# Chengyuann/AutoStyle-TTS

Hardware: AMD Instinct MI355X
Metric: synthesized audio sec/wall-sec (RTF^-1) + style-kNN QPS, IEMOCAP test batch (higher is better)
Workload: dtype f16; 1 GPU; BASELINE configs[1]: batch=8 utterances/GPU, kNN Q=8 x N=1000 x D=6144 k=3, synthesis Tt=32 Tp=150 Ts=250 (fixed-length decode, EOS ignored) -> 430 mel frames -> 110080 samples @ 22050 Hz; CosyVoice-300M shapes, random-init weights; parallelism=dp1 (model + bank replicated, utterances sharded, all-gather of style ids only)

## Files before the change

### autostyle-tts_amd/csrc/ops_tfm_fused.hip

```cpp
#include "common.h"
#include "xlane.h"

namespace astts {

static constexpr int TF_C = 256;
static constexpr int TF_DH = 64;
static constexpr int TF_KS = 72;
static constexpr int TF_AS = TF_C + 8;
static constexpr int TF_QROWS = 192;
static constexpr int TF_QS = 64;
static constexpr int TF_MAX_T = 384;

__device__ __forceinline__ int tf_q(int row, int col) { return row * TF_QS + ((((col >> 3) ^ row) & 7) << 3) + (col & 7); }

__device__ __forceinline__ float row16_sum(float v) {
    v += __builtin_bit_cast(float, __builtin_amdgcn_update_dpp(0, __builtin_bit_cast(int, v), 0x121, 0xf, 0xf, false));
    v += __builtin_bit_cast(float, __builtin_amdgcn_update_dpp(0, __builtin_bit_cast(int, v), 0x122, 0xf, 0xf, false));
    v += __builtin_bit_cast(float, __builtin_amdgcn_update_dpp(0, __builtin_bit_cast(int, v), 0x124, 0xf, 0xf, false));
    v += __builtin_bit_cast(float, __builtin_amdgcn_update_dpp(0, __builtin_bit_cast(int, v), 0x128, 0xf, 0xf, false));
    return v;
}

struct TfmAttnArgs {
    const float* x;
    const _Float16* w;
    const float* bias;
    const int* lens;
    _Float16* out;
    int b, heads, t;
    float eps, scale;
    int balance;
    const char* pf[3];
    unsigned pf_bytes[4];
};

template <bool FULL>
__device__ __forceinline__ void tfm_attn_body(const TfmAttnArgs& a, int* seq_out, int* unit_out) {
    extern __shared__ __attribute__((aligned(16))) _Float16 tf_smem[];
    const int tid = threadIdx.x, lane = tid & 63, wid = tid >> 6;
    const int c = lane & 31, hh = lane >> 5;
    int qs, head, b;
    {
        const int units = FULL ? a.heads : 2 * a.heads;
        const int L = blockIdx.x;
        int hq;
        if ((a.b & 7) == 0) {
            const int xcd = L & 7, slot = L >> 3;
            b = xcd + 8 * (slot / units);
            hq = slot % units;
        } else {
            b = L / units;
            hq = L % units;
        }
        head = FULL ? hq : hq >> 1;
        qs = FULL ? 0 : hq & 1;
    }
    const int T = a.t;
    const int nch = (T + 31) >> 5;
    const int tkp = nch * 32;
    const int vs = tkp + 4;
    const int hsplit = (nch + 1) / 2;
    const int pq0 = FULL ? 0 : (qs == 0 ? 0 : hsplit);
    const int pq1 = FULL ? nch : (qs == 0 ? hsplit : nch);
    _Float16* sK = tf_smem;
    _Float16* sVt = sK + (size_t)tkp * TF_KS;
    _Float16* sA = sVt + (size_t)TF_DH * vs;
    _Float16* sQ = sA + 2 * 32 * TF_AS;
    const float* xb = a.x + (int64_t)b * T * TF_C;
    const int hd = a.heads * TF_DH;

    const int role = wid >> 1;
    half8 wf[16];
    float bias_e[16];
    if (role < 3) {
        const int part = role == 0 ? 1 : (role == 1 ? 2 : 0);
        const int frow = part * hd + head * TF_DH + (wid & 1) * 32;
        const _Float16* wp = a.w + ((int64_t)(frow >> 5) * 16 * 64 + lane) * 8;
#pragma unroll
        for (int s = 0; s < 16; ++s) wf[s] = *reinterpret_cast<const half8*>(wp + (int64_t)s * 64 * 8);
#pragma unroll
        for (int e = 0; e < 16; ++e) {
            const int f = role == 1 ? c : (e & 3) + 8 * (e >> 2) + 4 * hh;
            bias_e[e] = a.bias ? a.bias[frow + f] : 0.0f;
        }
    }

    const int srow = tid >> 4, sseg = (tid & 15) * 16;
    constexpr int PF = 2;
    float4 xr[PF][4];
    auto load_chunk = [&](int ch, float4 (&r)[4]) {
        const int fr = min(ch * 32 + srow, T - 1);
        const float* p = xb + (int64_t)fr * TF_C + sseg;
#pragma unroll
        for (int i = 0; i < 4; ++i) r[i] = *reinterpret_cast<const float4*>(p + 4 * i);
    };
    auto stage_chunk = [&](int buf, const float4 (&r)[4]) {
        float s = 0.0f;
#pragma unroll
        for (int i = 0; i < 4; ++i) s += (r[i].x + r[i].y) + (r[i].z + r[i].w);
        s = row16_sum(s);
        const float mean = s * (1.0f / TF_C);
        float q = 0.0f;
#pragma unroll
        for (int i = 0; i < 4; ++i) {
            const float dx = r[i].x - mean, dy = r[i].y - mean, dz = r[i].z - mean, dw = r[i].w - mean;
            q += (dx * dx + dy * dy) + (dz * dz + dw * dw);
        }
        q = row16_sum(q);
        const float rstd = rsqrtf(q * (1.0f / TF_C) + a.eps);
        half8 h0, h1;
        h0[0] = (_Float16)((r[0].x - mean) * rstd); h0[1] = (_Float16)((r[0].y - mean) * rstd);
        h0[2] = (_Float16)((r[0].z - mean) * rstd); h0[3] = (_Float16)((r[0].w - mean) * rstd);
        h0[4] = (_Float16)((r[1].x - mean) * rstd); h0[5] = (_Float16)((r[1].y - mean) * rstd);
        h0[6] = (_Float16)((r[1].z - mean) * rstd); h0[7] = (_Float16)((r[1].w - mean) * rstd);
        h1[0] = (_Float16)((r[2].x - mean) * rstd); h1[1] = (_Float16)((r[2].y - mean) * rstd);
        h1[2] = (_Float16)((r[2].z - mean) * rstd); h1[3] = (_Float16)((r[2].w - mean) * rstd);
        h1[4] = (_Float16)((r[3].x - mean) * rstd); h1[5] = (_Float16)((r[3].y - mean) * rstd);
        h1[6] = (_Float16)((r[3].z - mean) * rstd); h1[7] = (_Float16)((r[3].w - mean) * rstd);
        _Float16* d = sA + (size_t)buf * 32 * TF_AS + srow * TF_AS + sseg;
        *reinterpret_cast<half8*>(d) = h0;
        *reinterpret_cast<half8*>(d + 8) = h1;
    };
    auto project_chunk = [&](int ch) {
        const int buf = ch & 1;
        const bool q_chunk = ch >= pq0 && ch < pq1;
        const bool q_parked = FULL && ch >= hsplit;
        const int qbase = FULL ? 0 : pq0;
        if (role < 2 || (role == 2 && q_chunk)) {
            const _Float16* ap = sA + (size_t)buf * 32 * TF_AS + c * TF_AS + 8 * hh;
            float16v acc;
#pragma unroll
            for (int e = 0; e < 16; ++e) acc[e] = bias_e[e];
            if (role == 1) {
#pragma unroll
                for (int s0 = 0; s0 < 16; s0 += 8) {
                    half8 af[8];
#pragma unroll
                    for (int s = 0; s < 8; ++s) af[s] = *reinterpret_cast<const half8*>(ap + 16 * (s0 + s));
#pragma unroll
                    for (int s = 0; s < 8; ++s) acc = __builtin_amdgcn_mfma_f32_32x32x16_f16(af[s], wf[s0 + s], acc, 0, 0, 0);
                }
                _Float16* vp = sVt + (size_t)((wid & 1) * 32 + c) * vs + ch * 32 + 4 * hh;
#pragma unroll
                for (int g = 0; g < 4; ++g) {
                    half4 h4;
                    h4[0] = (_Float16)acc[4 * g]; h4[1] = (_Float16)acc[4 * g + 1]; h4[2] = (_Float16)acc[4 * g + 2]; h4[3] = (_Float16)acc[4 * g + 3];
                    *reinterpret_cast<half4*>(vp + 8 * g) = h4;
                }
            } else {
#pragma unroll
                for (int s0 = 0; s0 < 16; s0 += 8) {
                    half8 af[8];
#pragma unroll
                    for (int s = 0; s < 8; ++s) af[s] = *reinterpret_cast<const half8*>(ap + 16 * (s0 + s));
#pragma unroll
                    for (int s = 0; s < 8; ++s) acc = __builtin_amdgcn_mfma_f32_32x32x16_f16(wf[s0 + s], af[s], acc, 0, 0, 0);
                }
                _Float16* kp = sK + (size_t)(ch * 32 + c) * TF_KS + (wid & 1) * 32 + 4 * hh;
                const int qr = (ch - qbase) * 32 + c;
                const int fr = ch * 32 + c;
                _Float16* park = a.out + ((int64_t)b * T + min(fr, T - 1)) * hd + head * TF_DH + (wid & 1) * 32 + 4 * hh;
#pragma unroll
                for (int g = 0; g < 4; ++g) {
                    half4 h4;
                    h4[0] = (_Float16)acc[4 * g]; h4[1] = (_Float16)acc[4 * g + 1]; h4[2] = (_Float16)acc[4 * g + 2]; h4[3] = (_Float16)acc[4 * g + 3];
                    if (role == 0) *reinterpret_cast<half4*>(kp + 8 * g) = h4;
                    else if (!q_parked) *reinterpret_cast<half4*>(sQ + tf_q(qr, (wid & 1) * 32 + 4 * hh + 8 * g)) = h4;
                    else if (fr < T) *reinterpret_cast<half4*>(park + 8 * g) = h4;
                }
            }
        }
    };
#pragma unroll
    for (int i = 0; i < PF; ++i)
        if (i < nch) load_chunk(i, xr[i]);
    stage_chunk(0, xr[0]);
    if (PF < nch) load_chunk(PF, xr[0]);
    __syncthreads();
    for (int ch0 = 0; ch0 < nch; ch0 += PF) {
#pragma unroll
        for (int u = 0; u < PF; ++u) {
            const int ch = ch0 + u;
            if (ch < nch) {
                if (ch + 1 < nch) stage_chunk((ch + 1) & 1, xr[(u + 1) % PF]);
                if (ch + 1 + PF < nch) load_chunk(ch + 1 + PF, xr[(u + 1) % PF]);
                project_chunk(ch);
                __syncthreads();
            }
        }
    }

    unsigned pf_keep[3];
    *seq_out = b;
    *unit_out = FULL ? head * 2 : head * 2 + qs;
    for (int hf = FULL ? 0 : qs; hf < (FULL ? 2 : qs + 1); ++hf) {
    const int qch0 = hf == 0 ? 0 : hsplit;
    const int qch1 = hf == 0 ? hsplit : nch;
    if (FULL && hf == 1) {
        __builtin_amdgcn_fence(__ATOMIC_RELEASE, "workgroup");
        __syncthreads();
        __builtin_amdgcn_fence(__ATOMIC_ACQUIRE, "workgroup");
        const int rows = (nch - hsplit) * 32;
        for (int i = tid; i < rows * 8; i += 512) {
            const int r = i >> 3, pc = i & 7;
            const int fr = min(hsplit * 32 + r, T - 1);
            const half8 v = *reinterpret_cast<const half8*>(a.out + ((int64_t)b * T + fr) * hd + head * TF_DH + pc * 8);
            *reinterpret_cast<half8*>(sQ + tf_q(r, pc * 8)) = v;
        }
        __syncthreads();
    }
    const int ntile = qch1 - qch0;
    int tile = -1, part = 0, parts = 1;
    if (wid < 4) {
        if (wid < ntile) tile = wid;
    } else if (!a.balance) {
        if (wid < ntile) tile = wid;
    } else if (ntile == 5) {
        tile = 4; part = wid - 4; parts = 4;
    } else if (ntile == 6) {
        tile = 4 + (wid & 1); part = (wid - 4) >> 1; parts = 2;
    }
    if (hf == (FULL ? 0 : qs)) {
        const unsigned slot = blockIdx.x >> 3, nslots = max(gridDim.x >> 3, 1u);
        asm volatile("" ::"s"(a.pf_bytes[3]));
#pragma unroll
        for (int r = 0; r < 3; ++r) {
            const unsigned lines = a.pf[r] ? (a.pf_bytes[r] + 127) >> 7 : 0u;
            const unsigned per = (lines + nslots - 1) / nslots;
            const unsigned ln = slot * per + tid;
            const char* base = a.pf[r] ? a.pf[r] : reinterpret_cast<const char*>(a.x);
            prefetch_line(base + (tid < per && ln < lines ? (size_t)ln << 7 : (size_t)0), pf_keep[r]);
        }
    }
    const int len = a.lens ? min(a.lens[b], T) : T;
    const int nkt = (len + 31) >> 5;
    const int jb0 = tile >= 0 ? (nkt * part / parts) * 32 : 0;
    const int jb1 = tile >= 0 ? min((nkt * (part + 1) / parts) * 32, len) : 0;
    const int tsafe = tile >= 0 ? tile : 0;
    const int q0 = (qch0 + tsafe) * 32;
    _Float16* qrow = sQ + (size_t)(tsafe * 32) * TF_QS;
    half8 qf[4];
    {
        const float qscale = a.scale * 1.44269504088896341f;
#pragma unroll
        for (int s = 0; s < 4; ++s) {
            const half8 raw = *reinterpret_cast<const half8*>(qrow + tf_q(c, 16 * s + 8 * hh));
#pragma unroll
            for (int i = 0; i < 8; ++i) qf[s][i] = (_Float16)((float)raw[i] * qscale);
        }
    }
    float16v ot[2];
#pragma unroll
    for (int e = 0; e < 16; ++e) {
        ot[0][e] = 0.0f;
        ot[1][e] = 0.0f;
    }
    float m_run = -INFINITY, l_run = 0.0f;
    for (int jb = jb0; jb < jb1; jb += 32) {
        float16v st;
#pragma unroll
        for (int e = 0; e < 16; ++e) st[e] = 0.0f;
        half8 kf[4];
        half4 vlo[4], vhi[4];
#pragma unroll
        for (int s = 0; s < 4; ++s) kf[s] = *reinterpret_cast<const half8*>(sK + (size_t)(jb + c) * TF_KS + 16 * s + 8 * hh);
#pragma unroll
        for (int dt = 0; dt < 2; ++dt)
#pragma unroll
            for (int s = 0; s < 2; ++s) {
                const _Float16* vrow = sVt + (size_t)(dt * 32 + c) * vs + jb + 16 * s + 4 * hh;
                vlo[dt * 2 + s] = *reinterpret_cast<const half4*>(vrow);
                vhi[dt * 2 + s] = *reinterpret_cast<const half4*>(vrow + 8);
            }
#pragma unroll
        for (int s = 0; s < 4; ++s) st = __builtin_amdgcn_mfma_f32_32x32x16_f16(kf[s], qf[s], st, 0, 0, 0);
        if (jb + 32 > len) {
#pragma unroll
            for (int e = 0; e < 16; ++e) {
                const int key = jb + (e & 3) + 8 * (e >> 2) + 4 * hh;
                st[e] = key < len ? st[e] : -INFINITY;
            }
        }
        float mloc = st[0];
#pragma unroll
        for (int e = 1; e < 16; ++e) mloc = fmaxf(mloc, st[e]);
        mloc = fmaxf(mloc, __shfl_xor(mloc, 32, 64));
        if (__builtin_amdgcn_ballot_w64(mloc > m_run) != 0) {
            const float m_new = fmaxf(m_run, mloc);
            const float alpha = __builtin_amdgcn_exp2f(m_run - m_new);
            l_run *= alpha;
            m_run = m_new;
#pragma unroll
            for (int e = 0; e < 16; ++e) {
                ot[0][e] *= alpha;
                ot[1][e] *= alpha;
            }
        }
        half8 pf[2];
#pragma unroll
        for (int e = 0; e < 16; ++e) {
            const float p = __builtin_amdgcn_exp2f(st[e] - m_run);
            l_run += p;
            pf[e >> 3][e & 7] = (_Float16)p;
        }
#pragma unroll
        for (int dt = 0; dt < 2; ++dt) {
#pragma unroll
            for (int s = 0; s < 2; ++s) {
                const half4 lo = vlo[dt * 2 + s], hi = vhi[dt * 2 + s];
                half8 vf;
                vf[0] = lo[0]; vf[1] = lo[1]; vf[2] = lo[2]; vf[3] = lo[3];
                vf[4] = hi[0]; vf[5] = hi[1]; vf[6] = hi[2]; vf[7] = hi[3];
                ot[dt] = __builtin_amdgcn_mfma_f32_32x32x16_f16(vf, pf[s], ot[dt], 0, 0, 0);
            }
        }
    }
    float* sM = reinterpret_cast<float*>(sA);
    if (part > 0) {
        float* mp = sM + (size_t)(ntile == 5 ? part - 1 : wid - 6) * 34 * 64 + lane;
#pragma unroll
        for (int e = 0; e < 16; ++e) {
            mp[e * 64] = ot[0][e];
            mp[(16 + e) * 64] = ot[1][e];
        }
        mp[32 * 64] = m_run;
        mp[33 * 64] = l_run;
    }
    __syncthreads();
    if (!(tile < 0 || part > 0)) {
    for (int hp = 1; hp < parts; ++hp) {
        const float* mp = sM + (size_t)(ntile == 5 ? hp - 1 : wid - 4) * 34 * 64 + lane;
        const float m_p = mp[32 * 64], l_p = mp[33 * 64];
        const float m_new = fmaxf(m_run, m_p);
        if (m_new > -INFINITY) {
            const float sa = __builtin_amdgcn_exp2f(m_run - m_new), sb = __builtin_amdgcn_exp2f(m_p - m_new);
#pragma unroll
            for (int e = 0; e < 16; ++e) {
                ot[0][e] = ot[0][e] * sa + mp[e * 64] * sb;
                ot[1][e] = ot[1][e] * sa + mp[(16 + e) * 64] * sb;
            }
            l_run = l_run * sa + l_p * sb;
            m_run = m_new;
        }
    }
    l_run += __shfl_xor(l_run, 32, 64);
    const float inv = l_run > 0.0f ? 1.0f / l_run : 0.0f;
#pragma unroll
    for (int dt = 0; dt < 2; ++dt)
#pragma unroll
        for (int g = 0; g < 4; ++g) {
            half4 h4;
            h4[0] = (_Float16)(ot[dt][4 * g] * inv); h4[1] = (_Float16)(ot[dt][4 * g + 1] * inv);
            h4[2] = (_Float16)(ot[dt][4 * g + 2] * inv); h4[3] = (_Float16)(ot[dt][4 * g + 3] * inv);
            *reinterpret_cast<half4*>(qrow + tf_q(c, dt * 32 + 8 * g + 4 * hh)) = h4;
        }
    __builtin_amdgcn_s_waitcnt(0xc07f);
    __builtin_amdgcn_wave_barrier();
#pragma unroll
    for (int i = 0; i < 4; ++i) {
        const int r = i * 8 + (lane >> 3), seg = (lane & 7) * 8;
        const int fr = q0 + r;
        if (fr < T)
            *reinterpret_cast<half8*>(a.out + ((int64_t)b * T + fr) * hd + head * TF_DH + seg) = *reinterpret_cast<const half8*>(qrow + tf_q(r, seg));
    }
    }
    }
    prefetch_keep(pf_keep[0]);
    prefetch_keep(pf_keep[1]);
    prefetch_keep(pf_keep[2]);
}

template <bool FULL>
__global__ __launch_bounds__(512, 2) void tfm_attn_fused(const float* p_x, const _Float16* p_w, const float* p_bias, const int* p_lens, int p_b, int p_heads,
                                                         int p_t, float p_eps, float p_scale, TfmAttnArgs a_in) {
    TfmAttnArgs a = a_in;
    a.x = p_x; a.w = p_w; a.bias = p_bias; a.lens = p_lens; a.b = p_b; a.heads = p_heads; a.t = p_t; a.eps = p_eps; a.scale = p_scale;
    int seq, unit;
    tfm_attn_body<FULL>(a, &seq, &unit);
}

__global__ void tfm_pack_frag(const _Float16* __restrict__ w, _Float16* __restrict__ out, int rows, int k) {
    const int64_t total = (int64_t)rows * k;
    const int ksteps = k >> 4;
    for (int64_t i = (int64_t)blockIdx.x * blockDim.x + threadIdx.x; i < total; i += (int64_t)gridDim.x * blockDim.x) {
        const int j = (int)(i & 7), ln = (int)((i >> 3) & 63);
        const int64_t q = i >> 9;
        const int s = (int)(q % ksteps);
        const int64_t tile = q / ksteps;
        out[i] = w[(tile * 32 + (ln & 31)) * k + 16 * s + 8 * (ln >> 5) + j];
    }
}

static constexpr int FF_HS = 256 + 8;

struct TfmFfnArgs {
    const float* x;
    const _Float16* w1;
    const float* b1;
    const _Float16* w2;
    const float* b2;
    float* out;
    const _Float16* attn;
    const _Float16* wo;
    const float* bo;
    int64_t m;
    int hidden, k0;
    float eps;
    const char* pf;
    unsigned pf_bytes;
};

template <bool WO>
__device__ __forceinline__ void tfm_ffn_body(const TfmFfnArgs& a, const int64_t m0, const int64_t mend, const unsigned rot_seed) {
    extern __shared__ __attribute__((aligned(16))) _Float16 tf_smem[];
    const int tid = threadIdx.x, lane = tid & 63, wid = tid >> 6;
    const int c = lane & 31, hh = lane >> 5;
    _Float16* sA = tf_smem;
    _Float16* sH = sA + 32 * TF_AS;
    float* sB1 = reinterpret_cast<float*>(sH + 2 * 32 * FF_HS);
    const int nchunk = a.hidden >> 8;
    const int ksteps2 = a.hidden >> 4;

    const int srow = tid >> 4, sseg = (tid & 15) * 4;
    float4 r[4];
    {
        const float* p = a.x + min(m0 + srow, mend - 1) * TF_C + sseg;
#pragma unroll
        for (int i = 0; i < 4; ++i) r[i] = *reinterpret_cast<const float4*>(p + 64 * i);
    }
    const int rot = (int)(rot_seed % (unsigned)nchunk);
    auto wrap = [&](int j) { return j >= nchunk ? j - nchunk : j; };
    half8 w1f[16], w2f[16];
    const _Float16* w1p = a.w1 + ((int64_t)wid * 16 * 64 + lane) * 8;
    const _Float16* w2p = a.w2 + ((int64_t)wid * ksteps2 * 64 + lane) * 8;
    auto load_w1 = [&](int j) {
        const _Float16* np = w1p + (int64_t)j * 8 * 16 * 512;
#pragma unroll
        for (int s = 0; s < 16; ++s) w1f[s] = *reinterpret_cast<const half8*>(np + (int64_t)s * 512);
    };
    auto load_w2 = [&](int j) {
        const _Float16* np = w2p + (int64_t)j * 16 * 512;
#pragma unroll
        for (int s = 0; s < 16; ++s) w2f[s] = *reinterpret_cast<const half8*>(np + (int64_t)s * 512);
    };
    float* sX = sB1 + a.hidden;
    if constexpr (WO) {
        const int as0 = a.k0 + 8;
        _Float16* sAtt = sH;
        const int nh = a.k0 >> 8;
        const _Float16* wop = a.wo + ((int64_t)wid * (a.k0 >> 4) * 64 + lane) * 8;
        half8 at[4];
        {
            const _Float16* p = a.attn + min(m0 + srow, mend - 1) * a.k0 + (tid & 15) * 8;
#pragma unroll
            for (int i = 0; i < 4; ++i)
                if (i * 128 < a.k0) at[i] = *reinterpret_cast<const half8*>(p + 128 * i);
        }
#pragma unroll
        for (int s = 0; s < 16; ++s) w2f[s] = *reinterpret_cast<const half8*>(wop + (int64_t)s * 512);
        load_w1(rot);
        for (int i = tid; i < a.hidden; i += 512) sB1[i] = a.b1 ? a.b1[i] : 0.0f;
        float16v acc0;
        {
            const float* bp = a.bo + wid * 32 + 4 * hh;
#pragma unroll
            for (int g = 0; g < 4; ++g) {
                const float4 b4 = a.bo ? *reinterpret_cast<const float4*>(bp + 8 * g) : make_float4(0.0f, 0.0f, 0.0f, 0.0f);
                acc0[4 * g] = b4.x; acc0[4 * g + 1] = b4.y; acc0[4 * g + 2] = b4.z; acc0[4 * g + 3] = b4.w;
            }
        }
#pragma unroll
        for (int i = 0; i < 4; ++i) *reinterpret_cast<float4*>(sX + srow * 260 + sseg + 64 * i) = r[i];
#pragma unroll
        for (int i = 0; i < 4; ++i)
            if (i * 128 < a.k0) *reinterpret_cast<half8*>(sAtt + srow * as0 + (tid & 15) * 8 + 128 * i) = at[i];
        __syncthreads();
        const _Float16* atp = sAtt + c * as0 + 8 * hh;
        for (int h = 0; h < nh; ++h) {
#pragma unroll
            for (int s0 = 0; s0 < 16; s0 += 8) {
                half8 af[8];
#pragma unroll
                for (int s = 0; s < 8; ++s) af[s] = *reinterpret_cast<const half8*>(atp + 16 * (16 * h + s0 + s));
#pragma unroll
                for (int s = 0; s < 8; ++s) acc0 = __builtin_amdgcn_mfma_f32_32x32x16_f16(w2f[s0 + s], af[s], acc0, 0, 0, 0);
            }
            if (h + 1 < nh) {
                const _Float16* np = wop + (int64_t)(h + 1) * 16 * 512;
#pragma unroll
                for (int s = 0; s < 16; ++s) w2f[s] = *reinterpret_cast<const half8*>(np + (int64_t)s * 512);
            }
        }
        load_w2(rot);
        {
            float* xp = sX + c * 260 + wid * 32 + 4 * hh;
#pragma unroll
            for (int g = 0; g < 4; ++g) {
                float4 v = *reinterpret_cast<float4*>(xp + 8 * g);
                v.x += acc0[4 * g]; v.y += acc0[4 * g + 1]; v.z += acc0[4 * g + 2]; v.w += acc0[4 * g + 3];
                *reinterpret_cast<float4*>(xp + 8 * g) = v;
            }
        }
        __syncthreads();
#pragma unroll
        for (int i = 0; i < 4; ++i) r[i] = *reinterpret_cast<const float4*>(sX + srow * 260 + sseg + 64 * i);
    } else {
        load_w1(rot);
        load_w2(rot);
        for (int i = tid; i < a.hidden; i += 512) sB1[i] = a.b1 ? a.b1[i] : 0.0f;
    }
    {
        float s = 0.0f;
#pragma unroll
        for (int i = 0; i < 4; ++i) s += (r[i].x + r[i].y) + (r[i].z + r[i].w);
        s = row16_sum(s);
        const float mean = s * (1.0f / TF_C);
        float q = 0.0f;
#pragma unroll
        for (int i = 0; i < 4; ++i) {
            const float dx = r[i].x - mean, dy = r[i].y - mean, dz = r[i].z - mean, dw = r[i].w - mean;
            q += (dx * dx + dy * dy) + (dz * dz + dw * dw);
        }
        q = row16_sum(q);
        const float rstd = rsqrtf(q * (1.0f / TF_C) + a.eps);
        _Float16* d = sA + srow * TF_AS + sseg;
#pragma unroll
        for (int i = 0; i < 4; ++i) {
            half4 h4;
            h4[0] = (_Float16)((r[i].x - mean) * rstd); h4[1] = (_Float16)((r[i].y - mean) * rstd);
            h4[2] = (_Float16)((r[i].z - mean) * rstd); h4[3] = (_Float16)((r[i].w - mean) * rstd);
            *reinterpret_cast<half4*>(d + 64 * i) = h4;
        }
    }
    __syncthreads();

    unsigned pf_keep;
    {
        const unsigned slot = blockIdx.x >> 3, nslots = max((gridDim.x + 7) >> 3, 1u);
        const unsigned lines = a.pf ? (a.pf_bytes + 127) >> 7 : 0u;
        const unsigned per = (lines + nslots - 1) / nslots;
        const unsigned ln = slot * per + tid;
        const char* base = a.pf ? a.pf : reinterpret_cast<const char*>(a.x);
        prefetch_line(base + (tid < per && ln < lines ? (size_t)ln << 7 : (size_t)0), pf_keep);
    }
    float16v acc2;
#pragma unroll
    for (int e = 0; e < 16; ++e) acc2[e] = 0.0f;
    const _Float16* ap = sA + c * TF_AS + 8 * hh;
    auto stage1 = [&](int j, float16v& acc1) {
        const float* bp = sB1 + (j * 8 + wid) * 32 + 4 * hh;
#pragma unroll
        for (int g = 0; g < 4; ++g) {
            const float4 b4 = *reinterpret_cast<const float4*>(bp + 8 * g);
            acc1[4 * g] = b4.x; acc1[4 * g + 1] = b4.y; acc1[4 * g + 2] = b4.z; acc1[4 * g + 3] = b4.w;
        }
#pragma unroll
        for (int s0 = 0; s0 < 16; s0 += 8) {
            half8 af[8];
#pragma unroll
            for (int s = 0; s < 8; ++s) af[s] = *reinterpret_cast<const half8*>(ap + 16 * (s0 + s));
#pragma unroll
            for (int s = 0; s < 8; ++s) acc1 = __builtin_amdgcn_mfma_f32_32x32x16_f16(w1f[s0 + s], af[s], acc1, 0, 0, 0);
        }
    };
    auto store_h = [&](int buf, const float (&gl)[16]) {
        _Float16* hp = sH + (size_t)buf * 32 * FF_HS + c * FF_HS + wid * 32 + 4 * hh;
#pragma unroll
        for (int g = 0; g < 4; ++g) {
            half4 h4;
            h4[0] = (_Float16)gl[4 * g]; h4[1] = (_Float16)gl[4 * g + 1]; h4[2] = (_Float16)gl[4 * g + 2]; h4[3] = (_Float16)gl[4 * g + 3];
            *reinterpret_cast<half4*>(hp + 8 * g) = h4;
        }
    };
    {
        float16v acc1;
        stage1(rot, acc1);
        if (nchunk > 1) load_w1(wrap(rot + 1));
        float gl[16];
#pragma unroll
        for (int e = 0; e < 16; ++e) gl[e] = gelu_erf_fast(acc1[e]);
        store_h(0, gl);
    }
    __syncthreads();
    for (int it = 0; it + 1 < nchunk; ++it) {
        const int jn = wrap(it + 1 + rot);
        float16v acc1;
        stage1(jn, acc1);
        if (it + 2 < nchunk) load_w1(wrap(jn + 1));
        const _Float16* hp = sH + (size_t)(it & 1) * 32 * FF_HS + c * FF_HS + 8 * hh;
        float gl[16];
#pragma unroll
        for (int s0 = 0; s0 < 16; s0 += 8) {
            half8 hf[8];
#pragma unroll
            for (int s = 0; s < 8; ++s) hf[s] = *reinterpret_cast<const half8*>(hp + 16 * (s0 + s));
            __builtin_amdgcn_sched_barrier(0);
#pragma unroll
            for (int s = 0; s < 8; ++s) {
                float gx = acc1[s0 + s];
                asm volatile("" : "+v"(hf[s]), "+v"(gx));
                acc2 = __builtin_amdgcn_mfma_f32_32x32x16_f16(hf[s], w2f[s0 + s], acc2, 0, 0, 0);
                float gy = gelu_erf_fast(gx);
                asm volatile("" : "+v"(gy), "+v"(hf[s]));
                gl[s0 + s] = gy;
                __builtin_amdgcn_sched_barrier(0);
            }
        }
        load_w2(jn);
        store_h((it + 1) & 1, gl);
        __syncthreads();
    }
    const int f = wid * 32 + c;
    float xr[16];
#pragma unroll
    for (int e = 0; e < 16; ++e) {
        const int re = (e & 3) + 8 * (e >> 2) + 4 * hh;
        xr[e] = WO ? sX[re * 260 + f] : a.x[min(m0 + re, mend - 1) * TF_C + f];
    }
    const float b2 = a.b2 ? a.b2[f] : 0.0f;
    {
        const _Float16* hp = sH + (size_t)((nchunk - 1) & 1) * 32 * FF_HS + c * FF_HS + 8 * hh;
#pragma unroll
        for (int s0 = 0; s0 < 16; s0 += 8) {
            half8 hf[8];
#pragma unroll
            for (int s = 0; s < 8; ++s) hf[s] = *reinterpret_cast<const half8*>(hp + 16 * (s0 + s));
#pragma unroll
            for (int s = 0; s < 8; ++s) acc2 = __builtin_amdgcn_mfma_f32_32x32x16_f16(hf[s], w2f[s0 + s], acc2, 0, 0, 0);
        }
    }
#pragma unroll
    for (int e = 0; e < 16; ++e) {
        const int64_t row = m0 + (e & 3) + 8 * (e >> 2) + 4 * hh;
        if (row < mend) a.out[row * TF_C + f] = (xr[e] + b2) + acc2[e];
    }
    prefetch_keep(pf_keep);
}

template <bool WO>
__global__ __launch_bounds__(512, 1) void tfm_ffn_fused(const float* p_x, const _Float16* p_w1, const _Float16* p_attn, const _Float16* p_wo, int64_t p_m,
                                                        int p_hidden, int p_k0, float p_eps, TfmFfnArgs a_in) {
    TfmFfnArgs a = a_in;
    a.x = p_x; a.w1 = p_w1; a.attn = p_attn; a.wo = p_wo; a.m = p_m; a.hidden = p_hidden; a.k0 = p_k0; a.eps = p_eps;
    const int64_t m0 = (int64_t)blockIdx.x * 32;
    tfm_ffn_body<WO>(a, m0, min(m0 + 32, a.m), blockIdx.x >> 3);
}

}

using namespace astts;

extern "C" {

int astts_op_tfm_pack_frag(const void* w_f16, void* out_f16, int32_t rows, int32_t k, astts_stream_t stream) {
    ASTTS_REQUIRE(w_f16 && out_f16 && w_f16 != out_f16, ASTTS_ERR_INVALID, "astts_op_tfm_pack_frag: null / aliased pointer");
    ASTTS_REQUIRE(k >= 16 && k % 16 == 0 && rows >= 32 && rows % 32 == 0, ASTTS_ERR_UNSUPPORTED,
                  "astts_op_tfm_pack_frag: rows=%d k=%d (rows must be a multiple of 32, k of 16)", rows, k);
    hipLaunchKernelGGL(tfm_pack_frag, dim3(256), dim3(256), 0, (hipStream_t)stream, (const _Float16*)w_f16, (_Float16*)out_f16, rows, k);
    ASTTS_CHECK_LAUNCH();
    return ASTTS_OK;
}

int astts_op_tfm_ffn_fused_supported(int32_t c, int32_t hidden) {
    return c == TF_C && hidden >= 256 && hidden % 256 == 0 && hidden <= 4096 ? 1 : 0;
}

int astts_op_tfm_ffn_fused(const float* x, const void* w1_frag_f16, const float* b1, const void* w2_frag_f16, const float* b2, float* out,
                           int64_t m, int32_t c, int32_t hidden, float eps, const void* attn_f16, const void* wo_frag_f16,
                           const float* bo, int32_t k0, const void* pf_ptr, uint32_t pf_bytes, astts_stream_t stream) {
    ASTTS_REQUIRE(x && w1_frag_f16 && w2_frag_f16 && out, ASTTS_ERR_INVALID, "astts_op_tfm_ffn_fused: null pointer");
    ASTTS_REQUIRE(astts_op_tfm_ffn_fused_supported(c, hidden), ASTTS_ERR_UNSUPPORTED,
                  "astts_op_tfm_ffn_fused: c=%d hidden=%d (channels 256, hidden a multiple of 256 <= 4096)", c, hidden);
    ASTTS_REQUIRE(m >= 1 && m <= ((int64_t)1 << 31) * 32 - 32 &&
                      (((uintptr_t)x | (uintptr_t)w1_frag_f16 | (uintptr_t)w2_frag_f16 | (uintptr_t)out) & 15) == 0,
                  ASTTS_ERR_INVALID, "astts_op_tfm_ffn_fused: m out of range or operands not 16-byte aligned");
    const bool wo = attn_f16 != nullptr;
    if (wo) {
        ASTTS_REQUIRE(wo_frag_f16 && (((uintptr_t)attn_f16 | (uintptr_t)wo_frag_f16 | (uintptr_t)bo) & 15) == 0, ASTTS_ERR_INVALID,
                      "astts_op_tfm_ffn_fused: attention rows without a projection weight, or operands not 16-byte aligned");
        ASTTS_REQUIRE(k0 == 256 || k0 == 512, ASTTS_ERR_UNSUPPORTED, "astts_op_tfm_ffn_fused: k0=%d (256 or 512)", k0);
    }
    static std::once_flag attr;
    std::call_once(attr, [] {
        (void)hipFuncSetAttribute(reinterpret_cast<const void*>(&tfm_ffn_fused<false>), hipFuncAttributeMaxDynamicSharedMemorySize, 96 * 1024);
        (void)hipFuncSetAttribute(reinterpret_cast<const void*>(&tfm_ffn_fused<true>), hipFuncAttributeMaxDynamicSharedMemorySize, 128 * 1024);
    });
    hipStream_t st = (hipStream_t)stream;
    const size_t lds = (size_t)(32 * TF_AS + 2 * 32 * FF_HS) * sizeof(_Float16) + (size_t)hidden * sizeof(float) + (wo ? 32 * 260 * sizeof(float) : 0);
    TfmFfnArgs a{x, (const _Float16*)w1_frag_f16, b1, (const _Float16*)w2_frag_f16, b2, out, (const _Float16*)attn_f16,
                 (const _Float16*)wo_frag_f16, bo, m, hidden, k0, eps, nullptr, 0u};
    static const bool pf_on = !(getenv("ASTTS_TFM_PREFETCH") && atoi(getenv("ASTTS_TFM_PREFETCH")) == 0);
    if (pf_ptr && pf_on) {
        a.pf = (const char*)pf_ptr;
        a.pf_bytes = pf_bytes;
    }
    const bool prof = prof_begin(ASTTS_PROF_GEMM_TILE, st, 4.0 * (double)m * TF_C * hidden + (wo ? 2.0 * (double)m * TF_C * k0 : 0.0));
    if (wo) hipLaunchKernelGGL(tfm_ffn_fused<true>, dim3((unsigned)((m + 31) / 32)), dim3(512), lds, st, a.x, a.w1, a.attn, a.wo, a.m, a.hidden, a.k0, a.eps, a);
    else hipLaunchKernelGGL(tfm_ffn_fused<false>, dim3((unsigned)((m + 31) / 32)), dim3(512), lds, st, a.x, a.w1, a.attn, a.wo, a.m, a.hidden, a.k0, a.eps, a);
    if (prof) prof_end(ASTTS_PROF_GEMM_TILE, st);
    ASTTS_CHECK_LAUNCH();
    return ASTTS_OK;
}

int astts_op_tfm_attn_fused_supported(int32_t c, int32_t heads, int32_t t) {
    return c == TF_C && heads >= 1 && heads <= 16 && t >= 1 && t <= TF_MAX_T ? 1 : 0;
}

int astts_op_tfm_attn_fused(const float* x, const void* wqkv_frag_f16, const float* bias, const int32_t* lens, void* out_f16, int32_t b,
                            int32_t heads, int32_t t, int32_t c, float eps, float scale, const void* const* pf_ptrs,
                            const uint32_t* pf_bytes, int32_t n_pf, astts_stream_t stream) {
    ASTTS_REQUIRE(n_pf >= 0 && n_pf <= 3 && (n_pf == 0 || (pf_ptrs && pf_bytes)), ASTTS_ERR_INVALID, "astts_op_tfm_attn_fused: n_pf=%d", n_pf);
    ASTTS_REQUIRE(x && wqkv_frag_f16 && out_f16, ASTTS_ERR_INVALID, "astts_op_tfm_attn_fused: null pointer");
    ASTTS_REQUIRE(astts_op_tfm_attn_fused_supported(c, heads, t), ASTTS_ERR_UNSUPPORTED,
                  "astts_op_tfm_attn_fused: c=%d heads=%d t=%d (channels 256, t <= %d)", c, heads, t, TF_MAX_T);
    ASTTS_REQUIRE(b >= 1 && (((uintptr_t)x | (uintptr_t)wqkv_frag_f16 | (uintptr_t)out_f16) & 15) == 0, ASTTS_ERR_INVALID,
                  "astts_op_tfm_attn_fused: operands must be 16-byte aligned");
    const int nch = (t + 31) / 32, tkp = nch * 32;
    const size_t lds = ((size_t)tkp * TF_KS + (size_t)TF_DH * (tkp + 4) + 2 * 32 * TF_AS + (size_t)TF_QROWS * TF_QS) * sizeof(_Float16);
    static std::once_flag attr;
    std::call_once(attr, [] {
        (void)hipFuncSetAttribute(reinterpret_cast<const void*>(&tfm_attn_fused<false>), hipFuncAttributeMaxDynamicSharedMemorySize, 160 * 1024);
        (void)hipFuncSetAttribute(reinterpret_cast<const void*>(&tfm_attn_fused<true>), hipFuncAttributeMaxDynamicSharedMemorySize, 160 * 1024);
    });
    TfmAttnArgs a{x, (const _Float16*)wqkv_frag_f16, bias, lens, (_Float16*)out_f16, b, heads, t, eps, scale, getenv("ASTTS_TFM_BALANCE") ? atoi(getenv("ASTTS_TFM_BALANCE")) : 1,
                  {nullptr, nullptr, nullptr}, {0u, 0u, 0u}};
    static const bool pf_on = !(getenv("ASTTS_TFM_PREFETCH") && atoi(getenv("ASTTS_TFM_PREFETCH")) == 0);
    for (int i = 0; i < n_pf && pf_on; ++i) {
        a.pf[i] = (const char*)pf_ptrs[i];
        a.pf_bytes[i] = pf_ptrs[i] ? pf_bytes[i] : 0u;
    }
    hipStream_t st = (hipStream_t)stream;
    const double flops = (double)b * heads * (3.0 * 2.0 * t * 64.0 * TF_C + 4.0 * (double)t * t * TF_DH);
    const bool prof = prof_begin(ASTTS_PROF_ATTN_FLASH, st, flops);
    const char* fe = getenv("ASTTS_TFM_ATTN_FULL");
    const int full_env = fe ? atoi(fe) : -1;
    const bool full = full_env >= 0 ? full_env != 0 : 2 * heads * b > 256;
    if (full) hipLaunchKernelGGL(tfm_attn_fused<true>, dim3(heads * b), dim3(512), lds, st, a.x, a.w, a.bias, a.lens, a.b, a.heads, a.t, a.eps, a.scale, a);
    else hipLaunchKernelGGL(tfm_attn_fused<false>, dim3(2 * heads * b), dim3(512), lds, st, a.x, a.w, a.bias, a.lens, a.b, a.heads, a.t, a.eps, a.scale, a);
    if (prof) prof_end(ASTTS_PROF_ATTN_FLASH, st);
    ASTTS_CHECK_LAUNCH();
    return ASTTS_OK;
}

}
```

Before: 478.0 audio-s/wall-s.

## Shrink fused attention LDS and registers to fit three blocks per CU

The fused LN+QKV+attention kernel drops the double-buffered staging tile and the 192-row Q LDS buffer. Each wave now pulls its Q tile straight into registers during projection, or reloads it from the parked global output for the second half. Per-lane bias arrays are replaced by on-demand loads, prefetch depth and the MFMA operand batch are halved, and launch bounds rise from 2 to 3 blocks per CU. The aim is higher occupancy and a smaller LDS footprint, at the cost of an extra barrier per chunk and less load prefetching.

```diff
diff --git a/autostyle-tts_amd/csrc/ops_tfm_fused.hip b/autostyle-tts_amd/csrc/ops_tfm_fused.hip
--- a/autostyle-tts_amd/csrc/ops_tfm_fused.hip
+++ b/autostyle-tts_amd/csrc/ops_tfm_fused.hip
@@ -7,7 +7,7 @@
 static constexpr int TF_DH = 64;
 static constexpr int TF_KS = 72;
 static constexpr int TF_AS = TF_C + 8;
-static constexpr int TF_QROWS = 192;
+static constexpr int TF_QTILES = 6;
 static constexpr int TF_QS = 64;
 static constexpr int TF_MAX_T = 384;
 
@@ -19,6 +19,17 @@
     v += __builtin_bit_cast(float, __builtin_amdgcn_update_dpp(0, __builtin_bit_cast(int, v), 0x124, 0xf, 0xf, false));
     v += __builtin_bit_cast(float, __builtin_amdgcn_update_dpp(0, __builtin_bit_cast(int, v), 0x128, 0xf, 0xf, false));
     return v;
+}
+
+__host__ __device__ constexpr int tf_scratch_bytes(int nch) {
+    const int h0 = (nch + 1) / 2, h1 = nch - h0;
+    const int slots = (h0 == 5 || h1 == 5) ? 3 : ((h0 == 6 || h1 == 6) ? 2 : 0);
+    const int stage = (32 * TF_AS + 2 * 32 * TF_QS) * 2, merge = slots * 34 * 64 * 4;
+    return stage > merge ? stage : merge;
+}
+__host__ __device__ constexpr size_t tf_attn_lds_bytes(int t, bool full) {
+    const int nch = (t + 31) / 32, tkp = nch * 32;
+    return ((size_t)tkp * TF_KS + (size_t)TF_DH * (tkp + 4)) * 2 + tf_scratch_bytes(nch) + (full ? (size_t)TF_QTILES * 32 * TF_QS * 2 : 0);
 }
 
 struct TfmAttnArgs {
@@ -37,7 +48,8 @@
 template <bool FULL>
 __device__ __forceinline__ void tfm_attn_body(const TfmAttnArgs& a, int* seq_out, int* unit_out) {
     extern __shared__ __attribute__((aligned(16))) _Float16 tf_smem[];
-    const int tid = threadIdx.x, lane = tid & 63, wid = tid >> 6;
+    const int tid = threadIdx.x, lane = tid & 63;
+    const int wid = __builtin_amdgcn_readfirstlane(tid >> 6);
     const int c = lane & 31, hh = lane >> 5;
     int qs, head, b;
     {
@@ -65,28 +77,26 @@
     _Float16* sK = tf_smem;
     _Float16* sVt = sK + (size_t)tkp * TF_KS;
     _Float16* sA = sVt + (size_t)TF_DH * vs;
-    _Float16* sQ = sA + 2 * 32 * TF_AS;
+    _Float16* sQ = sA + 32 * TF_AS;
+    _Float16* sT = FULL ? sA + tf_scratch_bytes(nch) / 2 : sK;
     const float* xb = a.x + (int64_t)b * T * TF_C;
     const int hd = a.heads * TF_DH;
 
     const int role = wid >> 1;
     half8 wf[16];
-    float bias_e[16];
+    typedef float float4u __attribute__((ext_vector_type(4), aligned(4)));
+    int bias_off = 0;
     if (role < 3) {
         const int part = role == 0 ? 1 : (role == 1 ? 2 : 0);
         const int frow = part * hd + head * TF_DH + (wid & 1) * 32;
         const _Float16* wp = a.w + ((int64_t)(frow >> 5) * 16 * 64 + lane) * 8;
 #pragma unroll
         for (int s = 0; s < 16; ++s) wf[s] = *reinterpret_cast<const half8*>(wp + (int64_t)s * 64 * 8);
-#pragma unroll
-        for (int e = 0; e < 16; ++e) {
-            const int f = role == 1 ? c : (e & 3) + 8 * (e >> 2) + 4 * hh;
-            bias_e[e] = a.bias ? a.bias[frow + f] : 0.0f;
-        }
+        bias_off = frow + (role == 1 ? c : 4 * hh);
     }
 
     const int srow = tid >> 4, sseg = (tid & 15) * 16;
-    constexpr int PF = 2;
+    constexpr int PF = 1;
     float4 xr[PF][4];
     auto load_chunk = [&](int ch, float4 (&r)[4]) {
         const int fr = min(ch * 32 + srow, T - 1);
@@ -94,7 +104,7 @@
 #pragma unroll
         for (int i = 0; i < 4; ++i) r[i] = *reinterpret_cast<const float4*>(p + 4 * i);
     };
-    auto stage_chunk = [&](int buf, const float4 (&r)[4]) {
+    auto norm_chunk = [&](const float4 (&r)[4], half8& h0, half8& h1) {
         float s = 0.0f;
 #pragma unroll
         for (int i = 0; i < 4; ++i) s += (r[i].x + r[i].y) + (r[i].z + r[i].w);
@@ -108,7 +118,6 @@
         }
         q = row16_sum(q);
         const float rstd = rsqrtf(q * (1.0f / TF_C) + a.eps);
-        half8 h0, h1;
         h0[0] = (_Float16)((r[0].x - mean) * rstd); h0[1] = (_Float16)((r[0].y - mean) * rstd);
         h0[2] = (_Float16)((r[0].z - mean) * rstd); h0[3] = (_Float16)((r[0].w - mean) * rstd);
         h0[4] = (_Float16)((r[1].x - mean) * rstd); h0[5] = (_Float16)((r[1].y - mean) * rstd);
@@ -117,28 +126,58 @@
         h1[2] = (_Float16)((r[2].z - mean) * rstd); h1[3] = (_Float16)((r[2].w - mean) * rstd);
         h1[4] = (_Float16)((r[3].x - mean) * rstd); h1[5] = (_Float16)((r[3].y - mean) * rstd);
         h1[6] = (_Float16)((r[3].z - mean) * rstd); h1[7] = (_Float16)((r[3].w - mean) * rstd);
-        _Float16* d = sA + (size_t)buf * 32 * TF_AS + srow * TF_AS + sseg;
+    };
+    auto put_chunk = [&](const half8& h0, const half8& h1) {
+        _Float16* d = sA + srow * TF_AS + sseg;
         *reinterpret_cast<half8*>(d) = h0;
         *reinterpret_cast<half8*>(d + 8) = h1;
     };
+    int tile = -1, part = 0, parts = 1;
+    auto assign_tile = [&](int ntile) {
+        tile = -1; part = 0; parts = 1;
+        if (wid < 4) {
+            if (wid < ntile) tile = wid;
+        } else if (!a.balance) {
+            if (wid < ntile) tile = wid;
+        } else if (ntile == 5) {
+            tile = 4; part = wid - 4; parts = 4;
+        } else if (ntile == 6) {
+            tile = 4 + (wid & 1); part = (wid - 4) >> 1; parts = 2;
+        }
+    };
+    const int hf0 = FULL ? 0 : qs;
+    const int qch0_first = hf0 == 0 ? 0 : hsplit;
+    half8 qf[4];
+#pragma unroll
+    for (int s = 0; s < 4; ++s)
+#pragma unroll
+        for (int i = 0; i < 8; ++i) qf[s][i] = (_Float16)0.0f;
+    const float qscale = a.scale * 1.44269504088896341f;
+    auto take_q = [&](const _Float16* rows) {
+#pragma unroll
+        for (int s = 0; s < 4; ++s) {
+            const half8 raw = *reinterpret_cast<const half8*>(rows + tf_q(c, 16 * s + 8 * hh));
+#pragma unroll
+            for (int i = 0; i < 8; ++i) qf[s][i] = (_Float16)((float)raw[i] * qscale);
+        }
+    };
     auto project_chunk = [&](int ch) {
-        const int buf = ch & 1;
         const bool q_chunk = ch >= pq0 && ch < pq1;
         const bool q_parked = FULL && ch >= hsplit;
-        const int qbase = FULL ? 0 : pq0;
         if (role < 2 || (role == 2 && q_chunk)) {
-            const _Float16* ap = sA + (size_t)buf * 32 * TF_AS + c * TF_AS + 8 * hh;
+            const _Float16* ap = sA + c * TF_AS + 8 * hh;
             float16v acc;
-#pragma unroll
-            for (int e = 0; e < 16; ++e) acc[e] = bias_e[e];
             if (role == 1) {
-#pragma unroll
-                for (int s0 = 0; s0 < 16; s0 += 8) {
-                    half8 af[8];
-#pragma unroll
-                    for (int s = 0; s < 8; ++s) af[s] = *reinterpret_cast<const half8*>(ap + 16 * (s0 + s));
-#pragma unroll
-                    for (int s = 0; s < 8; ++s) acc = __builtin_amdgcn_mfma_f32_32x32x16_f16(af[s], wf[s0 + s], acc, 0, 0, 0);
+                const float bias_v = a.bias ? a.bias[bias_off] : 0.0f;
+#pragma unroll
+                for (int e = 0; e < 16; ++e) acc[e] = bias_v;
+#pragma unroll
+                for (int s0 = 0; s0 < 16; s0 += 4) {
+                    half8 af[4];
+#pragma unroll
+                    for (int s = 0; s < 4; ++s) af[s] = *reinterpret_cast<const half8*>(ap + 16 * (s0 + s));
+#pragma unroll
+                    for (int s = 0; s < 4; ++s) acc = __builtin_amdgcn_mfma_f32_32x32x16_f16(af[s], wf[s0 + s], acc, 0, 0, 0);
                 }
                 _Float16* vp = sVt + (size_t)((wid & 1) * 32 + c) * vs + ch * 32 + 4 * hh;
 #pragma unroll
@@ -149,15 +188,21 @@
                 }
             } else {
 #pragma unroll
-                for (int s0 = 0; s0 < 16; s0 += 8) {
-                    half8 af[8];
-#pragma unroll
-                    for (int s = 0; s < 8; ++s) af[s] = *reinterpret_cast<const half8*>(ap + 16 * (s0 + s));
-#pragma unroll
-                    for (int s = 0; s < 8; ++s) acc = __builtin_amdgcn_mfma_f32_32x32x16_f16(wf[s0 + s], af[s], acc, 0, 0, 0);
+                for (int g = 0; g < 4; ++g) {
+                    float4u b4 = {0.0f, 0.0f, 0.0f, 0.0f};
+                    if (a.bias) b4 = *reinterpret_cast<const float4u*>(a.bias + bias_off + 8 * g);
+                    acc[4 * g] = b4[0]; acc[4 * g + 1] = b4[1]; acc[4 * g + 2] = b4[2]; acc[4 * g + 3] = b4[3];
+                }
+#pragma unroll
+                for (int s0 = 0; s0 < 16; s0 += 4) {
+                    half8 af[4];
+#pragma unroll
+                    for (int s = 0; s < 4; ++s) af[s] = *reinterpret_cast<const half8*>(ap + 16 * (s0 + s));
+#pragma unroll
+                    for (int s = 0; s < 4; ++s) acc = __builtin_amdgcn_mfma_f32_32x32x16_f16(wf[s0 + s], af[s], acc, 0, 0, 0);
                 }
                 _Float16* kp = sK + (size_t)(ch * 32 + c) * TF_KS + (wid & 1) * 32 + 4 * hh;
-                const int qr = (ch - qbase) * 32 + c;
+                const int qr = (ch & 1) * 32 + c;
                 const int fr = ch * 32 + c;
                 _Float16* park = a.out + ((int64_t)b * T + min(fr, T - 1)) * hd + head * TF_DH + (wid & 1) * 32 + 4 * hh;
 #pragma unroll
@@ -174,7 +219,12 @@
 #pragma unroll
     for (int i = 0; i < PF; ++i)
         if (i < nch) load_chunk(i, xr[i]);
-    stage_chunk(0, xr[0]);
+    assign_tile(hf0 == 0 ? hsplit : nch - hsplit);
+    {
+        half8 h0, h1;
+        norm_chunk(xr[0], h0, h1);
+        put_chunk(h0, h1);
+    }
     if (PF < nch) load_chunk(PF, xr[0]);
     __syncthreads();
     for (int ch0 = 0; ch0 < nch; ch0 += PF) {
@@ -182,10 +232,14 @@
         for (int u = 0; u < PF; ++u) {
             const int ch = ch0 + u;
             if (ch < nch) {
-                if (ch + 1 < nch) stage_chunk((ch + 1) & 1, xr[(u + 1) % PF]);
+                half8 h0, h1;
+                if (ch + 1 < nch) norm_chunk(xr[(u + 1) % PF], h0, h1);
                 if (ch + 1 + PF < nch) load_chunk(ch + 1 + PF, xr[(u + 1) % PF]);
                 project_chunk(ch);
                 __syncthreads();
+                if (ch + 1 < nch) put_chunk(h0, h1);
+                if (tile >= 0 && ch - qch0_first == tile) take_q(sQ + (size_t)(ch & 1) * 32 * TF_QS);
+                __syncthreads();
             }
         }
     }
@@ -193,32 +247,25 @@
     unsigned pf_keep[3];
     *seq_out = b;
     *unit_out = FULL ? head * 2 : head * 2 + qs;
-    for (int hf = FULL ? 0 : qs; hf < (FULL ? 2 : qs + 1); ++hf) {
+    for (int hf = hf0; hf < (FULL ? 2 : qs + 1); ++hf) {
     const int qch0 = hf == 0 ? 0 : hsplit;
     const int qch1 = hf == 0 ? hsplit : nch;
+    const int ntile = qch1 - qch0;
     if (FULL && hf == 1) {
         __builtin_amdgcn_fence(__ATOMIC_RELEASE, "workgroup");
         __syncthreads();
         __builtin_amdgcn_fence(__ATOMIC_ACQUIRE, "workgroup");
-        const int rows = (nch - hsplit) * 32;
-        for (int i = tid; i < rows * 8; i += 512) {
-            const int r = i >> 3, pc = i & 7;
-            const int fr = min(hsplit * 32 + r, T - 1);
-            const half8 v = *reinterpret_cast<const half8*>(a.out + ((int64_t)b * T + fr) * hd + head * TF_DH + pc * 8);
-            *reinterpret_cast<half8*>(sQ + tf_q(r, pc * 8)) = v;
-        }
-        __syncthreads();
-    }
-    const int ntile = qch1 - qch0;
-    int tile = -1, part = 0, parts = 1;
-    if (wid < 4) {
-        if (wid < ntile) tile = wid;
-    } else if (!a.balance) {
-        if (wid < ntile) tile = wid;
-    } else if (ntile == 5) {
-        tile = 4; part = wid - 4; parts = 4;
-    } else if (ntile == 6) {
-        tile = 4 + (wid & 1); part = (wid - 4) >> 1; parts = 2;
+        assign_tile(ntile);
+        if (tile >= 0) {
+            const int fr = min((hsplit + tile) * 32 + c, T - 1);
+            const _Float16* row = a.out + ((int64_t)b * T + fr) * hd + head * TF_DH;
+#pragma unroll
+            for (int s = 0; s < 4; ++s) {
+                const half8 raw = *reinterpret_cast<const half8*>(row + 16 * s + 8 * hh);
+#pragma unroll
+                for (int i = 0; i < 8; ++i) qf[s][i] = (_Float16)((float)raw[i] * qscale);
+            }
+        }
     }
     if (hf == (FULL ? 0 : qs)) {
         const unsigned slot = blockIdx.x >> 3, nslots = max(gridDim.x >> 3, 1u);
@@ -238,17 +285,7 @@
     const int jb1 = tile >= 0 ? min((nkt * (part + 1) / parts) * 32, len) : 0;
     const int tsafe = tile >= 0 ? tile : 0;
     const int q0 = (qch0 + tsafe) * 32;
-    _Float16* qrow = sQ + (size_t)(tsafe * 32) * TF_QS;
-    half8 qf[4];
-    {
-        const float qscale = a.scale * 1.44269504088896341f;
-#pragma unroll
-        for (int s = 0; s < 4; ++s) {
-            const half8 raw = *reinterpret_cast<const half8*>(qrow + tf_q(c, 16 * s + 8 * hh));
-#pragma unroll
-            for (int i = 0; i < 8; ++i) qf[s][i] = (_Float16)((float)raw[i] * qscale);
-        }
-    }
+    _Float16* qrow = sT + (size_t)(tsafe * 32) * TF_QS;
     float16v ot[2];
 #pragma unroll
     for (int e = 0; e < 16; ++e) {
@@ -371,7 +408,7 @@
 }
 
 template <bool FULL>
-__global__ __launch_bounds__(512, 2) void tfm_attn_fused(const float* p_x, const _Float16* p_w, const float* p_bias, const int* p_lens, int p_b, int p_heads,
+__global__ __launch_bounds__(512, 3) void tfm_attn_fused(const float* p_x, const _Float16* p_w, const float* p_bias, const int* p_lens, int p_b, int p_heads,
                                                          int p_t, float p_eps, float p_scale, TfmAttnArgs a_in) {
     TfmAttnArgs a = a_in;
     a.x = p_x; a.w = p_w; a.bias = p_bias; a.lens = p_lens; a.b = p_b; a.heads = p_heads; a.t = p_t; a.eps = p_eps; a.scale = p_scale;
@@ -715,8 +752,6 @@
                   "astts_op_tfm_attn_fused: c=%d heads=%d t=%d (channels 256, t <= %d)", c, heads, t, TF_MAX_T);
     ASTTS_REQUIRE(b >= 1 && (((uintptr_t)x | (uintptr_t)wqkv_frag_f16 | (uintptr_t)out_f16) & 15) == 0, ASTTS_ERR_INVALID,
                   "astts_op_tfm_attn_fused: operands must be 16-byte aligned");
-    const int nch = (t + 31) / 32, tkp = nch * 32;
-    const size_t lds = ((size_t)tkp * TF_KS + (size_t)TF_DH * (tkp + 4) + 2 * 32 * TF_AS + (size_t)TF_QROWS * TF_QS) * sizeof(_Float16);
     static std::once_flag attr;
     std::call_once(attr, [] {
         (void)hipFuncSetAttribute(reinterpret_cast<const void*>(&tfm_attn_fused<false>), hipFuncAttributeMaxDynamicSharedMemorySize, 160 * 1024);
@@ -735,6 +770,7 @@
     const char* fe = getenv("ASTTS_TFM_ATTN_FULL");
     const int full_env = fe ? atoi(fe) : -1;
     const bool full = full_env >= 0 ? full_env != 0 : 2 * heads * b > 256;
+    const size_t lds = tf_attn_lds_bytes(t, full);
     if (full) hipLaunchKernelGGL(tfm_attn_fused<true>, dim3(heads * b), dim3(512), lds, st, a.x, a.w, a.bias, a.lens, a.b, a.heads, a.t, a.eps, a.scale, a);
     else hipLaunchKernelGGL(tfm_attn_fused<false>, dim3(2 * heads * b), dim3(512), lds, st, a.x, a.w, a.bias, a.lens, a.b, a.heads, a.t, a.eps, a.scale, a);
     if (prof) prof_end(ASTTS_PROF_ATTN_FLASH, st);
```

Result: no change. 477.8 audio-s/wall-s (-0.1%).
